# aidagroup/quad-periodic-mpc

Hardware: AMD Instinct MI355X
Metric: QP solves/sec (N=10, 13-state, 12-force) at batch=65536; 1/2/4/8 GPU (higher is better)
Workload: dtype f32

## Files before the change

### quad-periodic-mpc_amd/csrc/cmpc_class1.hip

```cpp
#include <stdlib.h>

#include "cmpc_common.h"

#ifndef CMPC_W1_WAVES_60
#define CMPC_W1_WAVES_60 4
#endif
#ifndef CMPC_W1_WAVES_PER_EU
#define CMPC_W1_WAVES_PER_EU 4
#endif
#ifndef CMPC_C1_RL
#define CMPC_C1_RL 0
#endif
#ifndef CMPC_TRIP_PRIO_AT
#define CMPC_TRIP_PRIO_AT 0
#endif
#ifndef CMPC_C1_TRIP_PRIO
#define CMPC_C1_TRIP_PRIO 2
#endif
#ifndef C1_PIPE_GRP
#define C1_PIPE_GRP 4
#endif
#ifndef CMPC_C1_CHOL2
#define CMPC_C1_CHOL2 1
#endif
// ... 51 lines not shown
template <int NV>
struct C1Geo {
  static constexpr int NG = NV / 4;
  static constexpr int PSZ = 4 * NG * NV - 8 * NG * (NG - 1);
  __host__ __device__ static constexpr int prow(int r) {
    return 4 * (r >> 2) * NV - 8 * (r >> 2) * ((r >> 2) - 1) + (r & 3) * (NV - 4 * (r >> 2));
  }
  __host__ __device__ static constexpr int prow0(int r) { return prow(r) - (r & ~3); }
  __host__ __device__ static constexpr int tri(int r) { return r * NV - ((r * (r + 1)) >> 1); }
  static_assert(NV * NV - ((NV * (NV + 1)) >> 1) <= 4 * NG * NV - 8 * NG * (NG - 1), "exchange fits P");
};
__device__ __forceinline__ int rcol(int j) { return (j * (j + 1)) >> 1; }
constexpr int rinv_cols(int words) {
  int q = 0;
  while ((q + 1) * (q + 2) <= words) q++;
  return q;
}

constexpr int OFF_E = 0;
constexpr int OFF_ZE = OFF_E + 16 * MAXN;
constexpr int OFF_REC = OFF_ZE + 16 * MAXN;

constexpr int C1_MAXFS = 24;

template <int NV>
struct SharedC1 {
  static_assert(NV % 4 == 0 && NV <= NL, "row width");
  static_assert(NV * (NV + 1) / 2 <= C1Geo<NV>::PSZ, "R must fit in P");
  static_assert(OFF_REC + CMPC_REC_WORDS(MAXN) <= C1Geo<NV>::PSZ, "prep scratch must fit in P");
  static_assert(3 * C1_MAXFS >= NV, "stance list");
  static_assert(NV * (NV + 1) / 2 <= C1Geo<NV>::PSZ - NL, "vbuf in P's tail");
  __device__ __forceinline__ float* vbuf() { return &P[C1Geo<NV>::PSZ - NL]; }
  static constexpr int QI = rinv_cols(C1Geo<NV>::PSZ - NL);
  static constexpr int RB = C1Geo<NV>::PSZ - NL - QI * (QI + 1) / 2;
  static_assert(QI * (QI + 1) / 2 <= RB, "R and R^-1 side by side");
  float P[C1Geo<NV>::PSZ];
  union {
    float BdtT[12][16];
    float ibuf[NL];
    struct {
      float bufA[NL], bufB[NL];
      float cs[2 * NL];
    } gi;
  } u;
  float sub[C1_MAXFS];
  int sfs[C1_MAXFS];
  int blkbase[MAXN + 2];
  unsigned char varblk[NL], varcol[NL];
  unsigned char cmask[NL];
};

__device__ __forceinline__ void lsync() {
  __builtin_amdgcn_wave_barrier();
  asm volatile("" ::: "memory");
}

__device__ __forceinline__ float fdiv(float a, float b) { return a * fast_rcp(b); }

template <int M>
__device__ __forceinline__ void pin(float (&x)[M]) {
#pragma unroll
  for (int c = 0; c < M; c++) asm volatile("" : "+v"(x[c]));
}

template <int LO, int HI, int MA>
__device__ __forceinline__ float pick_col(const float (&x)[MA], int q) {
  static_assert(0 <= LO && LO < HI && HI <= MA, "column range");
  if constexpr (HI - LO == 1) {
    float r = x[LO];
    asm volatile("" : "+v"(r));
    return r;
  } else {
    constexpr int MID = (LO + HI) / 2;
    if (q < MID) return pick_col<LO, MID>(x, q);
    return pick_col<MID, HI>(x, q);
  }
}

#ifndef CMPC_FENCE_COLS
#define CMPC_FENCE_COLS 16
#endif
#define CMPC_SWEEP_FENCE(c)                                                                  \
  do {                                                                                       \
    if (((c) & (CMPC_FENCE_COLS - 1)) == CMPC_FENCE_COLS - 4) __builtin_amdgcn_sched_barrier(0); \
  } while (0)

template <int NV>
__device__ __forceinline__ void solve_c1(const float* __restrict__ rec, const KParams& P,
                                         SharedC1<NV>& sh, float* __restrict__ fout,
                                         uint8_t* __restrict__ st_out, int32_t* __restrict__ it_out,
                                         int* __restrict__ ovf_list, int* __restrict__ ovf_count,
                                         int inst) {
  using G = C1Geo<NV>;
  const int v = threadIdx.x;
  const int N = P.N;
#ifdef CMPC_PHASE_PROF
  unsigned long long ph[16] = {0, 0, 0, 0, 0, 0, 0, 0, 0, 0, 0, 0, 0, 0, 0, 0};
  unsigned long long t_sub = 0;
  unsigned long long t_last = clock64();
#endif
  {
    const float4* src = reinterpret_cast<const float4*>(rec);
    float4* dst = reinterpret_cast<float4*>(&sh.P[OFF_REC]);
    for (int t = v; t < (P.rec_words >> 2); t += 64) dst[t] = src[t];
  }
  lsync();
  const float* srec = &sh.P[OFF_REC];
  const unsigned char* gait = reinterpret_cast<const unsigned char*>(srec + CMPC_REC_HDR + 12 * N);
  int nfs = 0;
  unsigned long long msk0 = 0ull, msk1 = 0ull;
  for (int c0 = 0; c0 < 4 * N; c0 += 64) {
    const int t = c0 + v;
    float ub = 0.f;
    bool f = false;
    if (t < 4 * N) {
      ub = (float)gait[t] * P.f_max;
      f = !(ub < 0.01f && ub > -0.01f);
    }
    const unsigned long long m = __ballot(f);
    if (c0 == 0) msk0 = m; else msk1 = m;
    const int pre = __popcll(m & ((1ull << v) - 1ull));
    if (f && nfs + pre < C1_MAXFS) {
      sh.sfs[nfs + pre] = t;
      sh.sub[nfs + pre] = ub;
    }
    nfs += __popcll(m);
  }
  const int n = 3 * nfs;
  if (n > NV) {
    if (v == 0 && ovf_list) ovf_list[atomicAdd(ovf_count, 1)] = inst;
    return;
  }
  lsync();
  {
    int kb = 0, kc = 0;
    if (v < n) {
      const int fs = sh.sfs[v / 3];
      kb = fs >> 2;
      kc = 3 * (fs & 3) + v % 3;
    }
    sh.varblk[v] = (unsigned char)kb;
    sh.varcol[v] = (unsigned char)kc;
    if (v <= N) {
      const int b0 = 4 * v, b1 = 4 * v - 64;
      const unsigned long long lo = (b0 >= 64) ? msk0 : (msk0 & ((1ull << b0) - 1ull));
      const unsigned long long hi = (b1 <= 0) ? 0ull : (msk1 & ((1ull << b1) - 1ull));
      sh.blkbase[v] = 3 * (__popcll(lo) + __popcll(hi));
    }
    for (int t = v; t < nfs; t += 64) sh.cmask[t] = 0;
  }
  Model md;
  make_model(srec, P.dt, md);
  make_bdt<64>(srec, md, v, sh.u.BdtT);
  lsync();
  if (v < N) {
    float e[13];
    state_error(srec, md, v, srec + CMPC_REC_HDR + 12 * v, e);
#pragma unroll
    for (int j = 0; j < 13; j++) sh.P[OFF_E + 16 * v + j] = e[j];
  }
  lsync();
  float wts[13];
#pragma unroll
  for (int j = 0; j < 12; j++) wts[j] = P.wts[j];
  wts[12] = 0.f;
  {
    float ze[13];
#pragma unroll
    for (int j = 0; j < 13; j++) ze[j] = 0.f;
    for (int i = N - 1; i >= 0; i--) {
      float e[13];
#pragma unroll
      for (int j = 0; j < 13; j++) e[j] = sh.P[OFF_E + 16 * i + j];
      recur(md, wts, e, ze);
      float mine = 0.f;
#pragma unroll
      for (int j = 0; j < 13; j++) mine = (v == j) ? ze[j] : mine;
      if (v < 13) sh.P[OFF_ZE + 16 * i + v] = mine;
    }
  }
  lsync();
  C1_MARK(0);

  const bool real = v < n;
  float gv;
  {
    const int kv = real ? sh.varblk[v] : 0;
    const int cv = real ? sh.varcol[v] : 0;
    float b[13], u1[13], u2[13];
#pragma unroll
    for (int j = 0; j < 13; j++) b[j] = real ? sh.u.BdtT[cv][j] : 0.f;
    n1_mul(md, b, u1);
    n1_mul(md, u1, u2);
    {
      float zk[13];
#pragma unroll
      for (int j = 0; j < 13; j++) zk[j] = sh.P[OFF_ZE + 16 * kv + j];
      gv = real ? 2.f * dot13(b, zk) : 0.f;
    }
    lsync();
    const int myrow = G::tri(v);
    float z[13];
#pragma unroll
    for (int j = 0; j < 13; j++) z[j] = 0.f;
    for (int i = N - 1; i >= 0; i--) {
      const bool act = real && (i >= kv);
      const float k = (float)(i - kv);
      const float k2 = 0.5f * k * (k - 1.f);
      float gk[13];
#pragma unroll
      for (int j = 0; j < 13; j++) gk[j] = act ? fmaf(k2, u2[j], fmaf(k, u1[j], b[j])) : 0.f;
      recur(md, wts, gk, z);
      asm volatile("" ::: "memory");
      const int wb = __builtin_amdgcn_readfirstlane(sh.blkbase[i]);
      step_columns(sh.u.BdtT, step_mask(msk0, msk1, i), wb, z, [&](int w, float val) {
        if (w == v) val += P.alpha2;
        if (act && w >= v) sh.P[myrow + w] = val;
      });
    }
  }
  lsync();
  C1_MARK(1);

  float slot[NV + 1];
  {
    const int vv = (v < NV) ? v : 0;
    const int myrow = G::tri(vv);
    static_for<0, NV>([&](auto C) {
      constexpr int c = decltype(C)::value;
      const int addr = (c >= vv) ? myrow + c : G::tri(c) + vv;
      const float x = sh.P[addr];
      slot[c] = (real && c < n) ? x : ((c == v) ? 1.f : 0.f);
      if ((c & 7) == 7) __builtin_amdgcn_sched_barrier(0);
    });
    slot[NV] = gv;
  }
  lsync();

  int status = CMPC_OK;
  float my_inv = 1.f;
#if CMPC_C1_CHOL2
  float i0n = 1.f, betan = 0.f, i1n = 1.f, g0n = 0.f, g1n = 0.f;
  auto look = [&](auto JJ) {
    constexpr int j = decltype(JJ)::value, j1 = j + 1;
    constexpr int cj = j & ~3, cj1 = j1 & ~3;
    if constexpr (j1 < NV) {
    float d0 = rl(slot[j], j);
    const float h10 = rl(slot[j], j1);
    if (!(d0 > 0.f)) { status = CMPC_NOT_PD; d0 = 1e-30f; }
    i0n = __builtin_amdgcn_rsqf(d0);
    betan = h10 * (i0n * i0n);
    float d1 = fmaf(-h10, betan, rl(slot[j1], j1));
    if (!(d1 > 0.f)) { status = CMPC_NOT_PD; d1 = 1e-30f; }
    i1n = __builtin_amdgcn_rsqf(d1);
    g0n = rl(slot[NV], j);
    g1n = fmaf(-betan, g0n, rl(slot[NV], j1));
    const float s1 = fmaf(-slot[j], betan, slot[j1]);
#if CMPC_C1_FUSEDJ
    g0n = -g0n * i0n;
    g1n = -g1n * i1n;
    if (v >= cj && v < NV) sh.P[G::prow(j) + v - cj] = (v >= j) ? -slot[j] * i0n : 0.f;
    if (v >= cj1 && v < NV) sh.P[G::prow(j1) + v - cj1] = (v >= j1) ? -s1 * i1n : 0.f;
#else
    if (v >= cj && v < NV) sh.P[G::prow(j) + v - cj] = (v >= j) ? slot[j] : 0.f;
    if (v >= cj1 && v < NV) sh.P[G::prow(j1) + v - cj1] = (v >= j1) ? s1 : 0.f;
#endif
    lsync();
    }
  };
  if (n > 0) look(std::integral_constant<int, 0>{});
  float jc2 = 0.f, jc3 = 0.f;
  (void)jc2; (void)jc3;
  float xunc = 0.f;
  (void)xunc;
  static_for<0, NV / 2>([&](auto KB) {
    constexpr int k = 2 * decltype(KB)::value;
    constexpr int k1 = k + 1, k2 = k + 2;
    constexpr int c0 = k & ~3, c1 = k1 & ~3, c2 = k2 & ~3;
    constexpr int rk = G::prow(k), rk1 = G::prow(k1);
    if (k < n) {
      const float i0 = i0n, beta = betan, i1 = i1n, g0 = g0n, g1 = g1n;
#if CMPC_C1_FUSEDJ
      if (v == k) my_inv = i0;
      if (v == k1) my_inv = i1;
      const float s0 = slot[k];
      const float s1 = fmaf(-s0, beta, slot[k1]);
      const float a0 = (v > k) ? s0 * i0 : 0.f;
      const float a1 = (v > k1) ? s1 * i1 : 0.f;
#else
      if (v == k) { my_inv = i0; sh.u.ibuf[k] = i0; }
      if (v == k1) { my_inv = i1; sh.u.ibuf[k1] = i1; }
      const float s0 = slot[k];
      const float s1 = fmaf(-s0, beta, slot[k1]);
      const float a0 = (v > k) ? -s0 * (i0 * i0) : 0.f;
      const float a1 = (v > k1) ? -s1 * (i1 * i1) : 0.f;
#endif
      slot[NV] = fmaf(a1, g1, fmaf(a0, g0, slot[NV]));
      static_for<c2 / 4, NV / 4>([&](auto JC) {
        constexpr int c = 4 * decltype(JC)::value;
        const float4 r0 = *reinterpret_cast<const float4*>(&sh.P[rk + c - c0]);
        const float4 r1 = *reinterpret_cast<const float4*>(&sh.P[rk1 + c - c1]);
        axpy4(a0, r0, slot[c + 0], slot[c + 1], slot[c + 2], slot[c + 3]);
        axpy4(a1, r1, slot[c + 0], slot[c + 1], slot[c + 2], slot[c + 3]);
        if constexpr (k2 < NV && c == c2) {
          if (k2 < n) look(std::integral_constant<int, k2>{});
        }
        CMPC_SWEEP_FENCE(c);
      });
#if CMPC_C1_FUSEDJ == 2
      if constexpr ((k & 3) == 0) {
        f2v t0 = {(v == k) ? 1.f : 0.f, 0.f}, t1 = {(v == k1) ? 1.f : 0.f, 0.f};
        f2v t2 = {(v == k + 2) ? 1.f : 0.f, 0.f}, t3 = {(v == k + 3) ? 1.f : 0.f, 0.f};
#if CMPC_C1_JPIPE
        piped_sweep<0, k, 1>(
            [&](auto C) {
              constexpr int q = decltype(C)::value;
              return F4x4{*reinterpret_cast<const float4*>(&sh.P[G::prow(q) + k - q]),
                          *reinterpret_cast<const float4*>(&sh.P[G::prow(q + 1) + k - q]),
                          *reinterpret_cast<const float4*>(&sh.P[G::prow(q + 2) + k - q]),
                          *reinterpret_cast<const float4*>(&sh.P[G::prow(q + 3) + k - q])};
            },
            [&](auto C, F4x4 l) {
              constexpr int q = decltype(C)::value;
              const float4 la = l.a, lb = l.b, lc = l.c, ld = l.d;
#else
        static_for<0, k / 4>([&](auto QC) {
          constexpr int q = 4 * decltype(QC)::value;
          const float4 la = *reinterpret_cast<const float4*>(&sh.P[G::prow(q) + k - q]);
          const float4 lb = *reinterpret_cast<const float4*>(&sh.P[G::prow(q + 1) + k - q]);
          const float4 lc = *reinterpret_cast<const float4*>(&sh.P[G::prow(q + 2) + k - q]);
          const float4 ld = *reinterpret_cast<const float4*>(&sh.P[G::prow(q + 3) + k - q]);
#endif
          t0.x = fmaf(slot[q], la.x, t0.x); t1.x = fmaf(slot[q], la.y, t1.x);
          t2.x = fmaf(slot[q], la.z, t2.x); t3.x = fmaf(slot[q], la.w, t3.x);
          t0.y = fmaf(slot[q + 1], lb.x, t0.y); t1.y = fmaf(slot[q + 1], lb.y, t1.y);
          t2.y = fmaf(slot[q + 1], lb.z, t2.y); t3.y = fmaf(slot[q + 1], lb.w, t3.y);
          t0.x = fmaf(slot[q + 2], lc.x, t0.x); t1.x = fmaf(slot[q + 2], lc.y, t1.x);
          t2.x = fmaf(slot[q + 2], lc.z, t2.x); t3.x = fmaf(slot[q + 2], lc.w, t3.x);
          t0.y = fmaf(slot[q + 3], ld.x, t0.y); t1.y = fmaf(slot[q + 3], ld.y, t1.y);
          t2.y = fmaf(slot[q + 3], ld.z, t2.y); t3.y = fmaf(slot[q + 3], ld.w, t3.y);
#if CMPC_C1_JPIPE
            });
#else
          __builtin_amdgcn_sched_barrier(0);
        });
#endif
        const float hk = sh.P[G::prow(k) + k1 - (k & ~3)];
        const float xk = (t0.x + t0.y) * i0;
        slot[k] = xk;
        slot[k1] = fmaf(xk, hk, t1.x + t1.y) * i1;
#if CMPC_C1_XUNC
        xunc = fmaf(slot[k1], g1, fmaf(xk, g0, xunc));
#endif
        jc2 = t2.x + t2.y;
        jc3 = t3.x + t3.y;
        asm volatile("" : "+v"(jc2), "+v"(jc3));
      } else {
        constexpr int km = k - 2;
        const float2 l0 = *reinterpret_cast<const float2*>(&sh.P[G::prow(km) + k - (km & ~3)]);
        const float2 l1 = *reinterpret_cast<const float2*>(&sh.P[G::prow(km + 1) + k - (km & ~3)]);
        const float hk = sh.P[G::prow(k) + k1 - (k & ~3)];
        const float e0 = fmaf(slot[km + 1], l1.x, fmaf(slot[km], l0.x, jc2));
        const float e1 = fmaf(slot[km + 1], l1.y, fmaf(slot[km], l0.y, jc3));
        const float xk = e0 * i0;
        slot[k] = xk;
        slot[k1] = fmaf(xk, hk, e1) * i1;
#if CMPC_C1_XUNC
        xunc = fmaf(slot[k1], g1, fmaf(xk, g0, xunc));
// ... 485 lines not shown
```

### quad-periodic-mpc_amd/csrc/cmpc_common.h

```cpp
#pragma once
#include <hip/hip_runtime.h>
#include <stdint.h>

#include <type_traits>

#include "cmpc_kernels.h"

namespace cmpc {
namespace {

constexpr int MAXN = CMPC_MAX_HORIZON;
constexpr float kBigF = 3.0e38f;

__device__ __forceinline__ float rl(float x, int lane) {
  return __int_as_float(__builtin_amdgcn_readlane(__float_as_int(x), lane));
}
__device__ __forceinline__ int rli(int x, int lane) { return __builtin_amdgcn_readlane(x, lane); }

constexpr int kDppQuadSwap1 = 0xB1;
constexpr int kDppQuadSwap2 = 0x4E;
constexpr int kDppRowShl = 0x100;
constexpr int kDppRowShr = 0x110;
constexpr int kDppWaveShl1 = 0x130;
constexpr int kDppWaveShr1 = 0x138;
// ... 60 lines not shown
__device__ __forceinline__ float lane_next(float old, float v) { return dppf<kDppWaveShl1>(old, v); }
__device__ __forceinline__ int lane_next_i(int old, int v) { return dppi<kDppWaveShl1>(old, v); }

__device__ __forceinline__ int tid_opq() {
  int x = threadIdx.x;
  asm volatile("" : "+v"(x));
  return x;
}

#ifndef CMPC_LANE_ASM
#define CMPC_LANE_ASM 1
#endif
__device__ __forceinline__ int lane_opq() {
#if CMPC_LANE_ASM
  int x;
  asm volatile("v_mbcnt_lo_u32_b32 %0, -1, 0\n\tv_mbcnt_hi_u32_b32 %0, -1, %0" : "=v"(x));
#else
  int x = (int)__builtin_amdgcn_mbcnt_hi(~0u, __builtin_amdgcn_mbcnt_lo(~0u, 0u));
  asm volatile("" : "+v"(x));
#endif
  return x;
}

template <int I, int E, class F>
__device__ __forceinline__ void static_for(F&& f) {
  if constexpr (I < E) {
    f(std::integral_constant<int, I>{});
    static_for<I + 1, E>(f);
  }
}
template <int C0, int CE, int GRP, class Ld, class F>
__device__ __forceinline__ void piped_sweep(Ld&& ld, F&& f) {
  constexpr int NCH = (CE > C0) ? (CE - C0) / 4 : 0;
  if constexpr (NCH > 0) {
    using T = decltype(ld(std::integral_constant<int, C0>{}));
    constexpr int NG = (NCH + GRP - 1) / GRP;
    T cur[GRP], nxt[GRP];
    static_for<0, GRP>([&](auto I) {
      constexpr int ch = decltype(I)::value;
      if constexpr (ch < NCH) cur[ch] = ld(std::integral_constant<int, C0 + 4 * ch>{});
    });
    static_for<0, NG>([&](auto GI) {
      constexpr int g = decltype(GI)::value;
      static_for<0, GRP>([&](auto I) {
        constexpr int ch = (g + 1) * GRP + decltype(I)::value;
        if constexpr (ch < NCH) nxt[decltype(I)::value] = ld(std::integral_constant<int, C0 + 4 * ch>{});
      });
      __builtin_amdgcn_sched_barrier(0);
      static_for<0, GRP>([&](auto I) {
        constexpr int ch = g * GRP + decltype(I)::value;
        if constexpr (ch < NCH) f(std::integral_constant<int, C0 + 4 * ch>{}, cur[decltype(I)::value]);
      });
      __builtin_amdgcn_sched_barrier(0);
      static_for<0, GRP>([&](auto I) { cur[decltype(I)::value] = nxt[decltype(I)::value]; });
    });
  }
}
struct F4x2 {
  float4 a, b;
};
struct F4x4 {
  float4 a, b, c, d;
};

__device__ __forceinline__ float vopq(float x) {
  asm volatile("" : "+v"(x));
  return x;
}
__device__ __forceinline__ float sopq(float x) {
  asm volatile("" : "+s"(x));
  return x;
}
__device__ __forceinline__ float rfl(float x) {
  return __int_as_float(__builtin_amdgcn_readfirstlane(__float_as_int(x)));
}
__device__ __forceinline__ int opaque(int x) {
  x = __builtin_amdgcn_readfirstlane(x);
  asm volatile("" : "+s"(x));
  return x;
}
__device__ __forceinline__ float fast_rcp(float x) { return __builtin_amdgcn_rcpf(x); }

typedef float f2v __attribute__((ext_vector_type(2)));
__device__ __forceinline__ void axpy4(float a, float4 r, float& x0, float& x1, float& x2, float& x3) {
  x0 = fmaf(a, r.x, x0);
  x1 = fmaf(a, r.y, x1);
  x2 = fmaf(a, r.z, x2);
  x3 = fmaf(a, r.w, x3);
}
__device__ __forceinline__ void dot4(f2v& acc, float x0, float x1, float x2, float x3, float4 r) {
  acc.x = fmaf(x0, r.x, acc.x);
  acc.x = fmaf(x1, r.y, acc.x);
  acc.x = fmaf(x2, r.z, acc.x);
  acc.x = fmaf(x3, r.w, acc.x);
}
__device__ __forceinline__ void dot4x2(f2v& acc, float x0, float x1, float x2, float x3, float4 r) {
  acc.x = fmaf(x0, r.x, acc.x);
  acc.y = fmaf(x1, r.y, acc.y);
  acc.x = fmaf(x2, r.z, acc.x);
  acc.y = fmaf(x3, r.w, acc.y);
}

__device__ __forceinline__ void wsync() {
  __builtin_amdgcn_fence(__ATOMIC_RELEASE, "workgroup");
  __builtin_amdgcn_wave_barrier();
  __builtin_amdgcn_fence(__ATOMIC_ACQUIRE, "workgroup");
}

struct Model {
  float R[9];
  float n1r[9];
  float dt, dth, xdrag;
};

__device__ __forceinline__ void n1_mul(const Model& m, const float* x, float* y) {
#pragma unroll
  for (int i = 0; i < 3; i++) y[i] = m.n1r[i * 3 + 0] * x[6] + m.n1r[i * 3 + 1] * x[7] + m.n1r[i * 3 + 2] * x[8];
  y[3] = m.dt * x[9];
  y[4] = m.dt * x[10];
  y[5] = m.dt * x[11] + (m.dth * m.xdrag) * x[9] + m.dth * x[12];
#pragma unroll
  for (int i = 6; i < 11; i++) y[i] = 0.f;
  y[11] = (m.dt * m.xdrag) * x[9] + m.dt * x[12];
  y[12] = 0.f;
}

__device__ __forceinline__ void recur(const Model& m, const float* wts, const float* e, float* z) {
  float t[13];
#pragma unroll
  for (int j = 0; j < 13; j++) t[j] = z[j];
  const float c6 = m.n1r[0] * t[0] + m.n1r[3] * t[1] + m.n1r[6] * t[2];
  const float c7 = m.n1r[1] * t[0] + m.n1r[4] * t[1] + m.n1r[7] * t[2];
  const float c8 = m.n1r[2] * t[0] + m.n1r[5] * t[1] + m.n1r[8] * t[2];
  const float c9 = m.dt * t[3] + (m.dt * m.xdrag) * t[11] + (m.dth * m.xdrag) * t[5];
  const float c10 = m.dt * t[4];
  const float c11 = m.dt * t[5];
  const float c12 = m.dt * t[11] + m.dth * t[5];
#pragma unroll
  for (int j = 0; j < 13; j++) z[j] = wts[j] * e[j] + t[j];
  z[6] += c6; z[7] += c7; z[8] += c8; z[9] += c9; z[10] += c10; z[11] += c11; z[12] += c12;
}

__device__ __forceinline__ float dot13(const float* a, const float* b) {
  float s = 0.f;
#pragma unroll
  for (int j = 0; j < 13; j++) s = fmaf(a[j], b[j], s);
  return s;
}

__device__ __forceinline__ unsigned step_mask(unsigned long long m0, unsigned long long m1, int i) {
  return (unsigned)(((i < 16) ? (m0 >> (4 * i)) : (m1 >> (4 * i - 64))) & 15ull);
}

template <class St>
__device__ __forceinline__ void step_columns(const float (*BdtT)[16], unsigned mi, int wb,
                                             const float* z, St&& st) {
  int w = wb;
  static_for<0, 4>([&](auto F) {
    constexpr int f = decltype(F)::value;
    if (mi & (1u << f)) {
      static_for<0, 3>([&](auto A) {
        constexpr int c = 3 * f + decltype(A)::value;
        float bw[16];
#pragma unroll
        for (int q = 0; q < 4; q++) {
          const float4 b4 = *reinterpret_cast<const float4*>(&BdtT[c][4 * q]);
          bw[4 * q] = b4.x; bw[4 * q + 1] = b4.y; bw[4 * q + 2] = b4.z; bw[4 * q + 3] = b4.w;
        }
        st(w, 2.f * dot13(bw, z));
        w++;
      });
    }
  });
}

__device__ __forceinline__ void make_model(const float* __restrict__ rec, float dt, Model& md) {
  const float qw = rec[CMPC_REC_Q + 0], qx = rec[CMPC_REC_Q + 1], qy = rec[CMPC_REC_Q + 2],
              qz = rec[CMPC_REC_Q + 3];
  const float tx = 2.f * qx, ty = 2.f * qy, tz = 2.f * qz;
  const float twx = tx * qw, twy = ty * qw, twz = tz * qw;
  const float txx = tx * qx, txy = ty * qx, txz = tz * qx;
  const float tyy = ty * qy, tyz = tz * qy, tzz = tz * qz;
  md.R[0] = 1.f - (tyy + tzz); md.R[1] = txy - twz;         md.R[2] = txz + twy;
  md.R[3] = txy + twz;         md.R[4] = 1.f - (txx + tzz); md.R[5] = tyz - twx;
  md.R[6] = txz - twy;         md.R[7] = tyz + twx;         md.R[8] = 1.f - (txx + tyy);
  md.dt = dt;
  md.dth = dt * dt * 0.5f;
  md.xdrag = rec[CMPC_REC_XDRAG];
#pragma unroll
  for (int i = 0; i < 3; i++)
#pragma unroll
    for (int j = 0; j < 3; j++) md.n1r[i * 3 + j] = dt * md.R[j * 3 + i];
}

template <int NT>
__device__ __forceinline__ void make_bdt(const float* __restrict__ rec, const Model& md, int tid,
                                         float (*BdtT)[16]) {
  static_assert(NT >= 12, "one thread per force column");
  if (tid < 12) {
    const float Ib0 = .07f, Ib1 = 0.26f, Ib2 = 0.242f;
    float Iw[9];
#pragma unroll
    for (int i = 0; i < 3; i++)
#pragma unroll
      for (int j = 0; j < 3; j++)
        Iw[i * 3 + j] = md.R[i * 3 + 0] * Ib0 * md.R[j * 3 + 0] + md.R[i * 3 + 1] * Ib1 * md.R[j * 3 + 1] +
                        md.R[i * 3 + 2] * Ib2 * md.R[j * 3 + 2];
    const float c00 = Iw[4] * Iw[8] - Iw[5] * Iw[7];
    const float c10 = Iw[5] * Iw[6] - Iw[3] * Iw[8];
    const float c20 = Iw[3] * Iw[7] - Iw[4] * Iw[6];
    const float idet = 1.f / (Iw[0] * c00 + Iw[1] * c10 + Iw[2] * c20);
    float Ii[9];
    Ii[0] = c00 * idet; Ii[1] = (Iw[2] * Iw[7] - Iw[1] * Iw[8]) * idet; Ii[2] = (Iw[1] * Iw[5] - Iw[2] * Iw[4]) * idet;
    Ii[3] = c10 * idet; Ii[4] = (Iw[0] * Iw[8] - Iw[2] * Iw[6]) * idet; Ii[5] = (Iw[2] * Iw[3] - Iw[0] * Iw[5]) * idet;
    Ii[6] = c20 * idet; Ii[7] = (Iw[1] * Iw[6] - Iw[0] * Iw[7]) * idet; Ii[8] = (Iw[0] * Iw[4] - Iw[1] * Iw[3]) * idet;
    const float im = 1.f / 12.0f;
    const float dt = md.dt, dt2 = md.dth, dt3 = md.dt * md.dt * md.dt / 6.f;
    const int c = tid;
    const int b = c / 3, a = c - 3 * (c / 3);
    const float r0 = rec[CMPC_REC_R + 0 * 4 + b], r1 = rec[CMPC_REC_R + 1 * 4 + b],
                r2 = rec[CMPC_REC_R + 2 * 4 + b];
    const float cx0 = (a == 0) ? 0.f : (a == 1) ? -r2 : r1;
    const float cx1 = (a == 0) ? r2 : (a == 1) ? 0.f : -r0;
    const float cx2 = (a == 0) ? -r1 : (a == 1) ? r0 : 0.f;
    float T[3];
#pragma unroll
    for (int i = 0; i < 3; i++) T[i] = Ii[i * 3 + 0] * cx0 + Ii[i * 3 + 1] * cx1 + Ii[i * 3 + 2] * cx2;
    const float e0 = (a == 0) ? im : 0.f, e1 = (a == 1) ? im : 0.f, e2 = (a == 2) ? im : 0.f;
    float* col = BdtT[c];
#pragma unroll
    for (int s = 0; s < 3; s++)
      col[s] = dt2 * (md.R[0 * 3 + s] * T[0] + md.R[1 * 3 + s] * T[1] + md.R[2 * 3 + s] * T[2]);
    col[3] = dt2 * e0;
    col[4] = dt2 * e1;
    col[5] = dt2 * e2 + dt3 * md.xdrag * e0;
#pragma unroll
    for (int s = 0; s < 3; s++) col[6 + s] = dt * T[s];
    col[9] = dt * e0;
    col[10] = dt * e1;
    col[11] = dt * e2 + dt2 * md.xdrag * e0;
    col[12] = 0.f;
    col[13] = 0.f;
    col[14] = 0.f;
    col[15] = 0.f;
  }
}

template <typename RecPtr>
__device__ __forceinline__ void quat_to_rpy(RecPtr rec, float* rpy) {
  const float qw = rec[CMPC_REC_Q + 0], qx = rec[CMPC_REC_Q + 1], qy = rec[CMPC_REC_Q + 2],
              qz = rec[CMPC_REC_Q + 3];
  float as = -2.f * (qx * qz - qw * qy);
  as = fminf(as, 0.99999f);
  rpy[0] = atan2f(2.f * (qy * qz + qw * qx), qw * qw - qx * qx - qy * qy + qz * qz);
  rpy[1] = asinf(as);
  rpy[2] = atan2f(2.f * (qx * qy + qw * qz), qw * qw + qx * qx - qy * qy - qz * qz);
}

__device__ __forceinline__ void state_error(const float* __restrict__ rec, const Model& md, int i,
                                            const float* traj_i, float* e) {
  float x0[13];
  {
    quat_to_rpy(rec, x0);
#pragma unroll
    for (int k = 0; k < 3; k++) {
      x0[3 + k] = rec[CMPC_REC_P + k];
      x0[6 + k] = rec[CMPC_REC_W + k];
      x0[9 + k] = rec[CMPC_REC_V + k];
    }
    x0[12] = -9.8f;
  }
  float X1[13], X2[13], qf[13], F1[13], F2[13];
  n1_mul(md, x0, X1);
  n1_mul(md, X1, X2);
  const uint32_t flags = __float_as_uint(rec[CMPC_REC_FLAGS]);
  const float f3 = (flags & 1u) ? rec[CMPC_REC_FEST3] : 0.f;
#pragma unroll
  for (int j = 0; j < 13; j++) qf[j] = 0.f;
  qf[9] = md.dt * f3;
  qf[3] = md.dth * f3;
  qf[11] = md.dth * md.xdrag * f3;
  qf[5] = (md.dt * md.dt * md.dt / 6.f) * md.xdrag * f3;
  n1_mul(md, qf, F1);
  n1_mul(md, F1, F2);
  const float m1 = (float)(i + 1);
  const float m2 = 0.5f * m1 * (float)i;
  const float s2 = 0.5f * (float)i * (float)(i + 1);
  const float s3 = (float)(i + 1) * (float)i * (float)(i - 1) / 6.f;
#pragma unroll
  for (int j = 0; j < 13; j++) {
    float ev = x0[j] + m1 * X1[j] + m2 * X2[j] + m1 * qf[j] + s2 * F1[j] + s3 * F2[j];
    if (j < 12) ev -= traj_i[j];
    e[j] = ev;
  }
}

__device__ __forceinline__ double rl_d(double x, int lane) {
  const long long b = __double_as_longlong(x);
  const int lo = __builtin_amdgcn_readlane((int)b, lane);
  const int hi = __builtin_amdgcn_readlane((int)(b >> 32), lane);
  return __longlong_as_double(((long long)hi << 32) | (long long)(unsigned)lo);
}

struct Cons {
  int ia, iz;
  float ca, cb, bp;
};
__device__ __forceinline__ Cons decode_cons(int c, float mui, float sub_s) {
  Cons k;
  const int sft = c / 6, t = c - 6 * (c / 6);
  k.iz = 3 * sft + 2;
  if (t < 4) {
    k.ia = 3 * sft + (t >> 1);
    k.ca = (t & 1) ? -mui : mui;
    k.cb = 1.f;
    k.bp = 0.f;
  } else {
    k.ia = k.iz;
    k.ca = 0.f;
    k.cb = (t == 4) ? 1.f : -1.f;
    k.bp = (t == 4) ? 0.f : -sub_s;
  }
  return k;
}

}
}
```

### quad-periodic-mpc_amd/csrc/cmpc_condense.hip

```cpp
#include "cmpc_common.h"

namespace cmpc {
namespace {

constexpr int NTG = 256;

struct SharedC {
  float BdtT[12][16];
  float traj[12 * MAXN];
  float E[MAXN][16];
  float ZE[MAXN][16];
};

__device__ void condense_one(const float* __restrict__ rec, const KParams& P, SharedC& sh,
                             float* __restrict__ H, float* __restrict__ g) {
  const int tid = threadIdx.x;
  const int N = P.N;
  const int n = 12 * N;
  for (int t = tid; t < 12 * N; t += NTG) sh.traj[t] = rec[CMPC_REC_HDR + t];
  Model md;
  make_model(rec, P.dt, md);
  make_bdt<NTG>(rec, md, tid, sh.BdtT);
  __syncthreads();
  if (tid < N) {
    float e[13];
    state_error(rec, md, tid, &sh.traj[12 * tid], e);
#pragma unroll
    for (int j = 0; j < 13; j++) sh.E[tid][j] = e[j];
  }
  __syncthreads();
  float wts[13];
#pragma unroll
  for (int j = 0; j < 12; j++) wts[j] = P.wts[j];
  wts[12] = 0.f;
  if (tid < 64) {
    float ze[13];
#pragma unroll
    for (int j = 0; j < 13; j++) ze[j] = 0.f;
    for (int i = N - 1; i >= 0; i--) {
      float e[13];
#pragma unroll
      for (int j = 0; j < 13; j++) e[j] = sh.E[i][j];
      recur(md, wts, e, ze);
      if ((tid & 63) == 0) {
#pragma unroll
        for (int j = 0; j < 13; j++) sh.ZE[i][j] = ze[j];
      }
    }
  }
  __syncthreads();
  for (int v = tid; v < n; v += NTG) {
    const int kv = v / 12, cv = v - 12 * (v / 12);
    float b[13], u1[13], u2[13];
#pragma unroll
    for (int j = 0; j < 13; j++) b[j] = sh.BdtT[cv][j];
    n1_mul(md, b, u1);
    n1_mul(md, u1, u2);
    {
      float zk[13];
#pragma unroll
      for (int j = 0; j < 13; j++) zk[j] = sh.ZE[kv][j];
      g[v] = 2.f * dot13(b, zk);
    }
    float z[13];
#pragma unroll
    for (int j = 0; j < 13; j++) z[j] = 0.f;
    for (int i = N - 1; i >= kv; i--) {
      const float k = (float)(i - kv);
      const float k2 = 0.5f * k * (k - 1.f);
      float gk[13];
#pragma unroll
      for (int j = 0; j < 13; j++) gk[j] = fmaf(k2, u2[j], fmaf(k, u1[j], b[j]));
      recur(md, wts, gk, z);
      for (int w = max(12 * i, v); w < 12 * i + 12; w++) {
        float bw[13];
#pragma unroll
        for (int j = 0; j < 13; j++) bw[j] = sh.BdtT[w - 12 * i][j];
        float val = 2.f * dot13(bw, z);
        if (w == v) val += P.alpha2;
#ifdef CMPC_DIAG_PERTURB
        val *= 1.f + CMPC_DIAG_PERTURB;
#endif
        H[(size_t)v * n + w] = val;
        H[(size_t)w * n + v] = val;
      }
    }
  }
}

__global__ __launch_bounds__(NTG) void cmpc_condense_kernel(const float* __restrict__ recs, int batch, KParams P,
                                                            float* __restrict__ Hout, float* __restrict__ gout) {
  __shared__ SharedC sh;
  const size_t n = 12 * (size_t)P.N;
  for (int inst = blockIdx.x; inst < batch; inst += gridDim.x) {
    condense_one(recs + (size_t)inst * P.rec_words, P, sh, Hout + inst * n * n, gout + inst * n);
    __syncthreads();
  }
}

}

hipError_t launch_condense(const float* d_recs, int batch, const KParams& P, float* d_H, float* d_g,
                           hipStream_t stream) {
  if (batch <= 0) return hipSuccess;
  const int grid = batch < 2048 ? batch : 2048;
  hipLaunchKernelGGL(cmpc_condense_kernel, dim3(grid), dim3(NTG), 0, stream, d_recs, batch, P, d_H, d_g);
  return hipGetLastError();
}

}
```

### quad-periodic-mpc_amd/csrc/cmpc_tail.hip

```cpp
#include "cmpc_common.h"

#ifndef CMPC_TAIL_WAVES_PER_EU
#define CMPC_TAIL_WAVES_PER_EU 3
#endif
#ifndef CMPC_TRIP_PRIO_AT
#define CMPC_TRIP_PRIO_AT 0
#endif
#ifndef CMPC_TAIL_TRIP_PRIO
#define CMPC_TAIL_TRIP_PRIO 3
#endif
#ifndef CMPC_TAIL_DOT2
#define CMPC_TAIL_DOT2 0
#endif
#if CMPC_TAIL_DOT2
#define T_DOT dot4x2
#else
#define T_DOT dot4
#endif
#ifndef CMPC_TAIL_PRIO
#define CMPC_TAIL_PRIO 1
#endif
#ifndef TAIL_PIPE_GRP
#define TAIL_PIPE_GRP 4
#endif

#ifdef CMPC_PHASE_PROF
__device__ unsigned long long g_t_phase[16];
#define T_MARK(i)                               \
  do {                                          \
    const unsigned long long _n = clock64();    \
    ph[i] += _n - t_last;                       \
    t_last = _n;                                \
  } while (0)
#else
#define T_MARK(i) \
  do {            \
  } while (0)
#endif

namespace cmpc {
namespace {

constexpr int kTailRows = 8;

template <int T>
struct TGeo {
  static_assert(T == 8 || T == 16, "tail rows");
  static constexpr int NV = 64 + T;
  static constexpr int NG = NV / 4;
  static constexpr int PSZ = 4 * NG * NV - 8 * NG * (NG - 1);
  __host__ __device__ static constexpr int prow(int r) {
    return 4 * (r >> 2) * NV - 8 * (r >> 2) * ((r >> 2) - 1) + (r & 3) * (NV - 4 * (r >> 2));
  }
  __host__ __device__ static constexpr int tri(int r) { return r * NV - ((r * (r + 1)) >> 1); }
  static constexpr int LPR = 64 / T;
  static constexpr int TQ = T / LPR;
  static constexpr int SW = NV / LPR;
  static constexpr int MAXFS = (NV + 2) / 3;
  static_assert(NV * (NV + 1) / 2 <= PSZ, "exchange fits P");
  static_assert(64 * 65 / 2 <= PSZ - NV, "R (q <= 64) below vbuf");
};

constexpr int T_OFF_E = 0;
constexpr int T_OFF_ZE = T_OFF_E + 16 * MAXN;
constexpr int T_OFF_REC = T_OFF_ZE + 16 * MAXN;

__device__ __forceinline__ int rcol(int j) { return (j * (j + 1)) >> 1; }

constexpr int tail_rinv_cols(int words) {
  int q = 0;
  while ((q + 1) * (q + 2) <= words) q++;
  return q;
}

template <int T>
struct SharedT {
  using G = TGeo<T>;
  static_assert(T_OFF_REC + CMPC_REC_WORDS(MAXN) <= G::PSZ, "prep scratch must fit in P");
  __device__ __forceinline__ float* vbuf() { return &P[G::PSZ - G::NV]; }
  static constexpr int QI = tail_rinv_cols(G::PSZ - G::NV);
  static constexpr int RB = G::PSZ - G::NV - QI * (QI + 1) / 2;
  static_assert(QI * (QI + 1) / 2 <= RB, "R and R^-1 side by side");
  float P[G::PSZ];
  union {
    float BdtT[12][16];
    struct {
      float ibuf[G::NV];
      float bpair[G::NV / 2];
      float h22[T * T];
      float gt[T];
    } ch;
    struct {
      float bufA[G::NV], bufB[G::NV];
      float cs[2 * 64];
      float xs[G::NV];
    } gi;
  } u;
  float gtail[T];
  float sub[G::MAXFS];
  int sfs[G::MAXFS];
  int blkbase[MAXN + 2];
  unsigned char varblk[G::NV], varcol[G::NV];
  unsigned char cmask[G::MAXFS];
};

__device__ __forceinline__ void tsync() {
  __builtin_amdgcn_wave_barrier();
  asm volatile("" ::: "memory");
}

template <int M>
__device__ __forceinline__ void tpin(float (&x)[M]) {
#pragma unroll
  for (int c = 0; c < M; c++) asm volatile("" : "+v"(x[c]));
}

#define CMPC_TSWEEP_FENCE(c)                                       \
  do {                                                             \
    if (((c) & 15) == 12) __builtin_amdgcn_sched_barrier(0);       \
  } while (0)

template <int LPR>
__device__ __forceinline__ float group_sum(float v) {
  v += dppf<kDppQuadSwap1>(0.f, v);
  v += dppf<kDppQuadSwap2>(0.f, v);
  if constexpr (LPR == 8) v += dppf<kDppRowHalfMirror>(0.f, v);
  return v;
}

template <int T>
__device__ __forceinline__ void solve_t(const float* __restrict__ rec, const KParams& P,
                                        SharedT<T>& sh, float* __restrict__ fout,
                                        uint8_t* __restrict__ st_out, int32_t* __restrict__ it_out,
                                        int* __restrict__ ovf_list, int* __restrict__ ovf_count,
                                        int inst) {
  using G = TGeo<T>;
  constexpr int NV = G::NV, LPR = G::LPR, TQ = G::TQ, SW = G::SW;
  const int v = tid_opq();
  const int ti = v / LPR, ts = v % LPR;
  const int N = opaque(P.N);
#ifdef CMPC_PHASE_PROF
  unsigned long long ph[16] = {0, 0, 0, 0, 0, 0, 0, 0, 0, 0, 0, 0, 0, 0, 0, 0};
  unsigned long long t_last = clock64();
#endif
  {
    const float4* src = reinterpret_cast<const float4*>(rec);
    float4* dst = reinterpret_cast<float4*>(&sh.P[T_OFF_REC]);
    for (int t = v; t < (P.rec_words >> 2); t += 64) dst[t] = src[t];
  }
  tsync();
  const float* srec = &sh.P[T_OFF_REC];
  const unsigned char* gait = reinterpret_cast<const unsigned char*>(srec + CMPC_REC_HDR + 12 * N);
  int nfs = 0;
  unsigned long long msk0 = 0ull, msk1 = 0ull;
  for (int c0 = 0; c0 < 4 * N; c0 += 64) {
    const int t = c0 + v;
    float ub = 0.f;
    bool f = false;
    if (t < 4 * N) {
      ub = (float)gait[t] * P.f_max;
      f = !(ub < 0.01f && ub > -0.01f);
    }
    const unsigned long long m = __ballot(f);
    if (c0 == 0) msk0 = m; else msk1 = m;
    const int pre = __popcll(m & ((1ull << v) - 1ull));
    if (f && nfs + pre < G::MAXFS) {
      sh.sfs[nfs + pre] = t;
      sh.sub[nfs + pre] = ub;
    }
    nfs += __popcll(m);
  }
  const int n = 3 * nfs;
  if (n > NV || n <= 64) {
    if (v == 0) { st_out[0] = CMPC_BAD_INPUT; if (it_out) it_out[0] = 0; }
    return;
  }
  tsync();
  for (int t = v; t < NV; t += 64) {
    int kb = 0, kc = 0;
    if (t < n) {
      const int fs = sh.sfs[t / 3];
      kb = fs >> 2;
      kc = 3 * (fs & 3) + t % 3;
    }
    sh.varblk[t] = (unsigned char)kb;
    sh.varcol[t] = (unsigned char)kc;
  }
  if (v <= N) {
    const int b0 = 4 * v, b1 = 4 * v - 64;
    const unsigned long long lo = (b0 >= 64) ? msk0 : (msk0 & ((1ull << b0) - 1ull));
    const unsigned long long hi = (b1 <= 0) ? 0ull : (msk1 & ((1ull << b1) - 1ull));
    sh.blkbase[v] = 3 * (__popcll(lo) + __popcll(hi));
  }
  if (v < nfs) sh.cmask[v] = 0;
  Model md;
  make_model(srec, P.dt, md);
  make_bdt<64>(srec, md, v, sh.u.BdtT);
  tsync();
  if (v < N) {
    float e[13];
    state_error(srec, md, v, srec + CMPC_REC_HDR + 12 * v, e);
#pragma unroll
    for (int j = 0; j < 13; j++) sh.P[T_OFF_E + 16 * v + j] = e[j];
  }
  tsync();
  float wts[13];
#pragma unroll
  for (int j = 0; j < 12; j++) wts[j] = P.wts[j];
  wts[12] = 0.f;
  {
    float ze[13];
#pragma unroll
    for (int j = 0; j < 13; j++) ze[j] = 0.f;
    for (int i = N - 1; i >= 0; i--) {
      float e[13];
#pragma unroll
      for (int j = 0; j < 13; j++) e[j] = sh.P[T_OFF_E + 16 * i + j];
      recur(md, wts, e, ze);
      float mine = 0.f;
#pragma unroll
      for (int j = 0; j < 13; j++) mine = (v == j) ? ze[j] : mine;
      if (v < 13) sh.P[T_OFF_ZE + 16 * i + v] = mine;
    }
  }
  tsync();

  float gv;
  {
    const int kv = sh.varblk[v];
    const int cv = sh.varcol[v];
    float b[13], u1[13], u2[13];
#pragma unroll
    for (int j = 0; j < 13; j++) b[j] = sh.u.BdtT[cv][j];
    n1_mul(md, b, u1);
    n1_mul(md, u1, u2);
    {
      float zk[13];
#pragma unroll
      for (int j = 0; j < 13; j++) zk[j] = sh.P[T_OFF_ZE + 16 * kv + j];
      gv = 2.f * dot13(b, zk);
      const bool tr = v < T && 64 + v < n;
      const int kt = tr ? sh.varblk[64 + v] : 0, ct = tr ? sh.varcol[64 + v] : 0;
      float bt[13], zt[13];
#pragma unroll
      for (int j = 0; j < 13; j++) {
        bt[j] = sh.u.BdtT[ct][j];
        zt[j] = sh.P[T_OFF_ZE + 16 * kt + j];
      }
      const float gtl = tr ? 2.f * dot13(bt, zt) : 0.f;
      if (v < T) sh.gtail[v] = gtl;
    }
    tsync();
    const int myrow = G::tri(v);
    float z[13];
#pragma unroll
    for (int j = 0; j < 13; j++) z[j] = 0.f;
    for (int i = N - 1; i >= 0; i--) {
      const bool act = i >= kv;
      const float k = (float)(i - kv);
      const float k2 = 0.5f * k * (k - 1.f);
      float gk[13];
#pragma unroll
      for (int j = 0; j < 13; j++) gk[j] = act ? fmaf(k2, u2[j], fmaf(k, u1[j], b[j])) : 0.f;
      recur(md, wts, gk, z);
      asm volatile("" ::: "memory");
      const int wb = __builtin_amdgcn_readfirstlane(sh.blkbase[i]);
      step_columns(sh.u.BdtT, step_mask(msk0, msk1, i), wb, z, [&](int w, float val) {
        if (w == v) val += P.alpha2;
        if (act && w >= v) sh.P[myrow + w] = val;
      });
    }
  }
  {
    const int r = 64 + v;
    const bool real = v < T && r < n;
    const int kv = real ? sh.varblk[r] : 0;
    const int cv = real ? sh.varcol[r] : 0;
    const int k64 = __builtin_amdgcn_readfirstlane((int)sh.varblk[64]);
    float b[13], u1[13], u2[13];
#pragma unroll
    for (int j = 0; j < 13; j++) b[j] = sh.u.BdtT[cv][j];
    n1_mul(md, b, u1);
    n1_mul(md, u1, u2);
    const int myrow = G::tri(real ? r : 64);
    float z[13];
#pragma unroll
    for (int j = 0; j < 13; j++) z[j] = 0.f;
    for (int i = N - 1; i >= k64; i--) {
      const bool act = real && i >= kv;
      const float k = (float)(i - kv);
      const float k2 = 0.5f * k * (k - 1.f);
      float gk[13];
#pragma unroll
      for (int j = 0; j < 13; j++) gk[j] = act ? fmaf(k2, u2[j], fmaf(k, u1[j], b[j])) : 0.f;
      recur(md, wts, gk, z);
      asm volatile("" ::: "memory");
      const int wb = __builtin_amdgcn_readfirstlane(sh.blkbase[i]);
      step_columns(sh.u.BdtT, step_mask(msk0, msk1, i), wb, z, [&](int w, float val) {
        if (w == r) val += P.alpha2;
        if (act && w >= r) sh.P[myrow + w] = val;
      });
    }
  }
  tsync();

  T_MARK(0);
  float slot[NV + 1];
  {
    const int myrow = G::tri(v);
    static_for<0, NV>([&](auto C) {
      constexpr int c = decltype(C)::value;
      const int addr = (c >= v) ? myrow + c : G::tri(c) + v;
      const float x = sh.P[addr];
      if constexpr (c < 64) {
        slot[c] = x;
      } else {
        slot[c] = (c < opaque(n)) ? x : 0.f;
      }
      if ((c & 7) == 7) __builtin_amdgcn_sched_barrier(0);
    });
    slot[NV] = gv;
  }
  float tq[TQ];
  float gt;
  {
    const int r = 64 + ti;
#pragma unroll
    for (int m = 0; m < TQ; m++) {
      const int c = 64 + TQ * ts + m;
      const int addr = (c >= r) ? G::tri(r) + c : G::tri(c) + r;
      const float x = sh.P[addr];
      tq[m] = (r < n && c < n) ? x : ((r == c) ? 1.f : 0.f);
    }
    gt = (r < n) ? sh.gtail[ti] : 0.f;
  }
  tsync();

  T_MARK(1);
  int status = CMPC_OK;
  float my_inv = 1.f;
  float i0n = 1.f, betan = 0.f, i1n = 1.f, g0n = 0.f, g1n = 0.f;
  auto look = [&](auto JJ) {
    constexpr int j = decltype(JJ)::value, j1 = j + 1;
    constexpr int cj = j & ~3, cj1 = j1 & ~3;
    if constexpr (j1 < 64) {
      float d0 = rl(slot[j], j);
      const float h10 = rl(slot[j], j1);
      if (!(d0 > 0.f)) { status = CMPC_NOT_PD; d0 = 1e-30f; }
      i0n = __builtin_amdgcn_rsqf(d0);
      betan = h10 * (i0n * i0n);
      float d1 = fmaf(-h10, betan, rl(slot[j1], j1));
      if (!(d1 > 0.f)) { status = CMPC_NOT_PD; d1 = 1e-30f; }
      i1n = __builtin_amdgcn_rsqf(d1);
      g0n = rl(slot[NV], j);
      g1n = fmaf(-betan, g0n, rl(slot[NV], j1));
      const float s1 = fmaf(-slot[j], betan, slot[j1]);
      if (v >= cj) sh.P[G::prow(j) + v - cj] = (v >= j) ? slot[j] : 0.f;
      if (v >= cj1) sh.P[G::prow(j1) + v - cj1] = (v >= j1) ? s1 : 0.f;
      tsync();
    }
  };
  auto pub_tail = [&](auto JJ) {
    constexpr int j = decltype(JJ)::value, j1 = j + 1;
    constexpr int bj = G::prow(j) + 64 - (j & ~3), bj1 = G::prow(j1) + 64 - (j1 & ~3);
    {
      float x = 0.f;
      static_for<0, T>([&](auto M) {
        constexpr int m = decltype(M)::value;
        const float a = rl(slot[64 + m], j), b = rl(slot[64 + m], j1);
        x = (v == m) ? a : x;
        x = (v == T + m) ? b : x;
      });
      if (v < 2 * T) sh.P[(v < T) ? bj + v : bj1 + v - T] = x;
    }
  };
  look(std::integral_constant<int, 0>{});
  pub_tail(std::integral_constant<int, 0>{});
  tsync();
  static_for<0, 32>([&](auto KB) {
    constexpr int k = 2 * decltype(KB)::value;
    constexpr int k1 = k + 1, k2 = k + 2;
    constexpr int c0 = k & ~3, c1 = k1 & ~3, c2 = k2 & ~3;
    constexpr int rk = G::prow(k), rk1 = G::prow(k1);
    const float i0 = i0n, beta = betan, i1 = i1n, g0 = g0n, g1 = g1n;
    if (v == k) { my_inv = i0; sh.u.ch.ibuf[k] = i0; }
    if (v == k1) { my_inv = i1; sh.u.ch.ibuf[k1] = i1; }
    if (v == 0) sh.u.ch.bpair[k / 2] = beta;
    const float s0 = slot[k];
    const float s1 = fmaf(-s0, beta, slot[k1]);
    const float a0 = (v > k) ? -s0 * (i0 * i0) : 0.f;
    const float a1 = (v > k1) ? -s1 * (i1 * i1) : 0.f;
    slot[NV] = fmaf(a1, g1, fmaf(a0, g0, slot[NV]));
    static_for<c2 / 4, 16>([&](auto JC) {
      constexpr int c = 4 * decltype(JC)::value;
      const float4 r0 = *reinterpret_cast<const float4*>(&sh.P[rk + c - c0]);
      const float4 r1 = *reinterpret_cast<const float4*>(&sh.P[rk1 + c - c1]);
      axpy4(a0, r0, slot[c + 0], slot[c + 1], slot[c + 2], slot[c + 3]);
      axpy4(a1, r1, slot[c + 0], slot[c + 1], slot[c + 2], slot[c + 3]);
      if constexpr (k2 < 64 && c == c2) look(std::integral_constant<int, k2>{});
      CMPC_TSWEEP_FENCE(c);
    });
    tpin(slot);
    {
      const float a0t = fmaf(-beta, a1, a0);
      static_for<16, NV / 4>([&](auto JC) {
        constexpr int c = 4 * decltype(JC)::value;
        const float4 r0 = *reinterpret_cast<const float4*>(&sh.P[rk + c - c0]);
        const float4 r1 = *reinterpret_cast<const float4*>(&sh.P[rk1 + c - c1]);
        axpy4(a0t, r0, slot[c + 0], slot[c + 1], slot[c + 2], slot[c + 3]);
        axpy4(a1, r1, slot[c + 0], slot[c + 1], slot[c + 2], slot[c + 3]);
      });
      tpin(slot);
      const float h0 = sh.P[rk + 64 + ti - c0], h1 = sh.P[rk1 + 64 + ti - c1];
      const float s1t = fmaf(-h0, beta, h1);
      const float a1r = -s1t * (i1 * i1);
      const float a0c = -h0 * (i0 * i0);
      const float a0r = fmaf(-beta, a1r, a0c);
#pragma unroll
      for (int m = 0; m < TQ; m++) {
        const float p0 = sh.P[rk + 64 + TQ * ts + m - c0], p1 = sh.P[rk1 + 64 + TQ * ts + m - c1];
        tq[m] = fmaf(a1r, p1, fmaf(a0r, p0, tq[m]));
      }
      gt = fmaf(a1r, g1, fmaf(a0c, g0, gt));
    }
    if constexpr (k2 < 64) pub_tail(std::integral_constant<int, k2>{});
    tsync();
    tpin(slot);
    tpin(tq);
    asm volatile("" : "+v"(gt));
  });

  T_MARK(2);
  float yt = 0.f;
  {
#pragma unroll
    for (int m = 0; m < TQ; m++) sh.u.ch.h22[ti * T + TQ * ts + m] = tq[m];
    if (ts == 0) sh.u.ch.gt[ti] = gt;
    tsync();
    float trow[T];
    const int li = (v < T) ? v : 0;
    static_for<0, T>([&](auto C) {
      constexpr int c = decltype(C)::value;
      trow[c] = (v < T) ? sh.u.ch.h22[li * T + c] : 0.f;
    });
    float gti = (v < T) ? sh.u.ch.gt[li] : 0.f;
    float tinv = 1.f;
    tsync();
    static_for<0, T>([&](auto TT) {
      constexpr int t = decltype(TT)::value;
      constexpr int k = 64 + t, ck = k & ~3, rk = G::prow(k);
      if (v < T && v >= ck - 64) sh.P[rk + 64 + v - ck] = (v >= t) ? trow[t] : 0.f;
// ... 555 lines not shown
```

Measured before the change: 48.17 million.

## Compute Hessian step entries via structured B projection instead of dense dot13

Replaces the per-column 13-element dot products against the shared-memory B matrix with a factored form. It projects z once per step through the rotation, inverse inertia and mass terms, then forms each force column's three entries with a cross product against foot positions. It also exploits sparsity in the column-power expansion (col_power) so that only the nonzero terms of u1/u2 are used. Shared-memory loads and FMAs per Hessian entry drop, at the cost of extra per-thread registers for CondGeo and possible float rounding differences. The tail kernel keeps the old dot13 path by default.

```diff
diff --git a/quad-periodic-mpc_amd/csrc/cmpc_class1.hip b/quad-periodic-mpc_amd/csrc/cmpc_class1.hip
--- a/quad-periodic-mpc_amd/csrc/cmpc_class1.hip
+++ b/quad-periodic-mpc_amd/csrc/cmpc_class1.hip
@@ -227,6 +227,8 @@
   Model md;
   make_model(srec, P.dt, md);
   make_bdt<64>(srec, md, v, sh.u.BdtT);
+  CondGeo cg;
+  make_cond_geo<true>(srec, md, cg);
   lsync();
   if (v < N) {
     float e[13];
@@ -283,12 +285,13 @@
       const float k = (float)(i - kv);
       const float k2 = 0.5f * k * (k - 1.f);
       float gk[13];
-#pragma unroll
-      for (int j = 0; j < 13; j++) gk[j] = act ? fmaf(k2, u2[j], fmaf(k, u1[j], b[j])) : 0.f;
+      col_power(b, u1, u2, k, k2, gk);
+#pragma unroll
+      for (int j = 0; j < 13; j++) gk[j] = act ? gk[j] : 0.f;
       recur(md, wts, gk, z);
       asm volatile("" ::: "memory");
       const int wb = __builtin_amdgcn_readfirstlane(sh.blkbase[i]);
-      step_columns(sh.u.BdtT, step_mask(msk0, msk1, i), wb, z, [&](int w, float val) {
+      step_entries(md, cg, sh.u.BdtT, step_mask(msk0, msk1, i), wb, z, [&](int w, float val) {
         if (w == v) val += P.alpha2;
         if (act && w >= v) sh.P[myrow + w] = val;
       });
diff --git a/quad-periodic-mpc_amd/csrc/cmpc_common.h b/quad-periodic-mpc_amd/csrc/cmpc_common.h
--- a/quad-periodic-mpc_amd/csrc/cmpc_common.h
+++ b/quad-periodic-mpc_amd/csrc/cmpc_common.h
@@ -236,9 +236,100 @@
   return (unsigned)(((i < 16) ? (m0 >> (4 * i)) : (m1 >> (4 * i - 64))) & 15ull);
 }
 
+#ifndef CMPC_COND_DOT13
+#define CMPC_COND_DOT13 0
+#endif
+
+struct CondGeo {
+  float Ii[9];
+  float r[12];
+};
+struct StepProj {
+  float w[3], p[3];
+};
+
+__device__ __forceinline__ void make_iinv(const Model& md, float* Ii) {
+  const float Ib0 = .07f, Ib1 = 0.26f, Ib2 = 0.242f;
+  float Iw[9];
+#pragma unroll
+  for (int i = 0; i < 3; i++)
+#pragma unroll
+    for (int j = 0; j < 3; j++)
+      Iw[i * 3 + j] = md.R[i * 3 + 0] * Ib0 * md.R[j * 3 + 0] + md.R[i * 3 + 1] * Ib1 * md.R[j * 3 + 1] +
+                      md.R[i * 3 + 2] * Ib2 * md.R[j * 3 + 2];
+  const float c00 = Iw[4] * Iw[8] - Iw[5] * Iw[7];
+  const float c10 = Iw[5] * Iw[6] - Iw[3] * Iw[8];
+  const float c20 = Iw[3] * Iw[7] - Iw[4] * Iw[6];
+  const float idet = 1.f / (Iw[0] * c00 + Iw[1] * c10 + Iw[2] * c20);
+  Ii[0] = c00 * idet; Ii[1] = (Iw[2] * Iw[7] - Iw[1] * Iw[8]) * idet; Ii[2] = (Iw[1] * Iw[5] - Iw[2] * Iw[4]) * idet;
+  Ii[3] = c10 * idet; Ii[4] = (Iw[0] * Iw[8] - Iw[2] * Iw[6]) * idet; Ii[5] = (Iw[2] * Iw[3] - Iw[0] * Iw[5]) * idet;
+  Ii[6] = c20 * idet; Ii[7] = (Iw[1] * Iw[6] - Iw[0] * Iw[7]) * idet; Ii[8] = (Iw[0] * Iw[4] - Iw[1] * Iw[3]) * idet;
+}
+
+template <bool UNIFORM, typename RecPtr>
+__device__ __forceinline__ void make_cond_geo(RecPtr rec, const Model& md, CondGeo& cg) {
+  make_iinv(md, cg.Ii);
+#pragma unroll
+  for (int j = 0; j < 12; j++) cg.r[j] = rec[CMPC_REC_R + j];
+  if constexpr (UNIFORM) {
+#pragma unroll
+    for (int j = 0; j < 9; j++) cg.Ii[j] = rfl(cg.Ii[j]);
+#pragma unroll
+    for (int j = 0; j < 12; j++) cg.r[j] = rfl(cg.r[j]);
+  }
+}
+
+__device__ __forceinline__ void step_proj(const Model& md, const CondGeo& cg, const float* z, StepProj& pj) {
+  const float dt2 = 2.f * md.dt, dtq = 2.f * md.dth, dtc = md.dt * md.dt * md.dt / 3.f;
+  const float im = 1.f / 12.0f;
+  float q[3];
+#pragma unroll
+  for (int i = 0; i < 3; i++)
+    q[i] = fmaf(dt2, z[6 + i], dtq * fmaf(md.R[i * 3 + 2], z[2], fmaf(md.R[i * 3 + 1], z[1], md.R[i * 3] * z[0])));
+#pragma unroll
+  for (int j = 0; j < 3; j++)
+    pj.w[j] = fmaf(cg.Ii[6 + j], q[2], fmaf(cg.Ii[3 + j], q[1], cg.Ii[j] * q[0]));
+#pragma unroll
+  for (int a = 0; a < 3; a++) pj.p[a] = im * fmaf(dt2, z[9 + a], dtq * z[3 + a]);
+  pj.p[0] = fmaf(im * md.xdrag, fmaf(dtq, z[11], dtc * z[5]), pj.p[0]);
+}
+
+__device__ __forceinline__ void foot_entries(const StepProj& pj, float r0, float r1, float r2, float* out) {
+  out[0] = fmaf(pj.w[1], r2, fmaf(-pj.w[2], r1, pj.p[0]));
+  out[1] = fmaf(pj.w[2], r0, fmaf(-pj.w[0], r2, pj.p[1]));
+  out[2] = fmaf(pj.w[0], r1, fmaf(-pj.w[1], r0, pj.p[2]));
+}
+
+__device__ __forceinline__ void col_power(const float* b, const float* u1, const float* u2, float k, float k2,
+                                          float* e) {
+#pragma unroll
+  for (int j = 0; j < 5; j++) e[j] = fmaf(k, u1[j], b[j]);
+  e[5] = fmaf(k2, u2[5], fmaf(k, u1[5], b[5]));
+#pragma unroll
+  for (int j = 6; j < 11; j++) e[j] = b[j];
+  e[11] = fmaf(k, u1[11], b[11]);
+  e[12] = b[12];
+}
+
 template <class St>
-__device__ __forceinline__ void step_columns(const float (*BdtT)[16], unsigned mi, int wb,
-                                             const float* z, St&& st) {
+__device__ __forceinline__ void step_columns(const CondGeo& cg, unsigned mi, int wb, const StepProj& pj,
+                                             St&& st) {
+  int w = wb;
+  static_for<0, 4>([&](auto F) {
+    constexpr int f = decltype(F)::value;
+    if (mi & (1u << f)) {
+      float val[3];
+      foot_entries(pj, cg.r[f], cg.r[4 + f], cg.r[8 + f], val);
+      st(w, val[0]);
+      st(w + 1, val[1]);
+      st(w + 2, val[2]);
+      w += 3;
+    }
+  });
+}
+template <class St>
+__device__ __forceinline__ void step_columns_dot13(const float (*BdtT)[16], unsigned mi, int wb,
+                                                   const float* z, St&& st) {
   int w = wb;
   static_for<0, 4>([&](auto F) {
     constexpr int f = decltype(F)::value;
@@ -256,6 +347,17 @@
       });
     }
   });
+}
+template <class St>
+__device__ __forceinline__ void step_entries(const Model& md, const CondGeo& cg, const float (*BdtT)[16],
+                                             unsigned mi, int wb, const float* z, St&& st) {
+#if CMPC_COND_DOT13
+  step_columns_dot13(BdtT, mi, wb, z, st);
+#else
+  StepProj pj;
+  step_proj(md, cg, z, pj);
+  step_columns(cg, mi, wb, pj, st);
+#endif
 }
 
 __device__ __forceinline__ void make_model(const float* __restrict__ rec, float dt, Model& md) {
@@ -282,22 +384,8 @@
                                          float (*BdtT)[16]) {
   static_assert(NT >= 12, "one thread per force column");
   if (tid < 12) {
-    const float Ib0 = .07f, Ib1 = 0.26f, Ib2 = 0.242f;
-    float Iw[9];
-#pragma unroll
-    for (int i = 0; i < 3; i++)
-#pragma unroll
-      for (int j = 0; j < 3; j++)
-        Iw[i * 3 + j] = md.R[i * 3 + 0] * Ib0 * md.R[j * 3 + 0] + md.R[i * 3 + 1] * Ib1 * md.R[j * 3 + 1] +
-                        md.R[i * 3 + 2] * Ib2 * md.R[j * 3 + 2];
-    const float c00 = Iw[4] * Iw[8] - Iw[5] * Iw[7];
-    const float c10 = Iw[5] * Iw[6] - Iw[3] * Iw[8];
-    const float c20 = Iw[3] * Iw[7] - Iw[4] * Iw[6];
-    const float idet = 1.f / (Iw[0] * c00 + Iw[1] * c10 + Iw[2] * c20);
     float Ii[9];
-    Ii[0] = c00 * idet; Ii[1] = (Iw[2] * Iw[7] - Iw[1] * Iw[8]) * idet; Ii[2] = (Iw[1] * Iw[5] - Iw[2] * Iw[4]) * idet;
-    Ii[3] = c10 * idet; Ii[4] = (Iw[0] * Iw[8] - Iw[2] * Iw[6]) * idet; Ii[5] = (Iw[2] * Iw[3] - Iw[0] * Iw[5]) * idet;
-    Ii[6] = c20 * idet; Ii[7] = (Iw[1] * Iw[6] - Iw[0] * Iw[7]) * idet; Ii[8] = (Iw[0] * Iw[4] - Iw[1] * Iw[3]) * idet;
+    make_iinv(md, Ii);
     const float im = 1.f / 12.0f;
     const float dt = md.dt, dt2 = md.dth, dt3 = md.dt * md.dt * md.dt / 6.f;
     const int c = tid;
diff --git a/quad-periodic-mpc_amd/csrc/cmpc_condense.hip b/quad-periodic-mpc_amd/csrc/cmpc_condense.hip
--- a/quad-periodic-mpc_amd/csrc/cmpc_condense.hip
+++ b/quad-periodic-mpc_amd/csrc/cmpc_condense.hip
@@ -21,6 +21,8 @@
   Model md;
   make_model(rec, P.dt, md);
   make_bdt<NTG>(rec, md, tid, sh.BdtT);
+  CondGeo cg;
+  make_cond_geo<true>(rec, md, cg);
   __syncthreads();
   if (tid < N) {
     float e[13];
@@ -69,21 +71,18 @@
       const float k = (float)(i - kv);
       const float k2 = 0.5f * k * (k - 1.f);
       float gk[13];
-#pragma unroll
-      for (int j = 0; j < 13; j++) gk[j] = fmaf(k2, u2[j], fmaf(k, u1[j], b[j]));
+      col_power(b, u1, u2, k, k2, gk);
       recur(md, wts, gk, z);
-      for (int w = max(12 * i, v); w < 12 * i + 12; w++) {
-        float bw[13];
-#pragma unroll
-        for (int j = 0; j < 13; j++) bw[j] = sh.BdtT[w - 12 * i][j];
-        float val = 2.f * dot13(bw, z);
+      step_entries(md, cg, sh.BdtT, 15u, 12 * i, z, [&](int w, float val) {
         if (w == v) val += P.alpha2;
 #ifdef CMPC_DIAG_PERTURB
         val *= 1.f + CMPC_DIAG_PERTURB;
 #endif
-        H[(size_t)v * n + w] = val;
-        H[(size_t)w * n + v] = val;
-      }
+        if (w >= v) {
+          H[(size_t)v * n + w] = val;
+          H[(size_t)w * n + v] = val;
+        }
+      });
     }
   }
 }
diff --git a/quad-periodic-mpc_amd/csrc/cmpc_tail.hip b/quad-periodic-mpc_amd/csrc/cmpc_tail.hip
--- a/quad-periodic-mpc_amd/csrc/cmpc_tail.hip
+++ b/quad-periodic-mpc_amd/csrc/cmpc_tail.hip
@@ -1,3 +1,7 @@
+
+#ifndef CMPC_COND_DOT13
+#define CMPC_COND_DOT13 1
+#endif
 #include "cmpc_common.h"
 
 #ifndef CMPC_TAIL_WAVES_PER_EU
@@ -225,6 +229,8 @@
   }
   tsync();
 
+  CondGeo cg;
+  make_cond_geo<true>(srec, md, cg);
   float gv;
   {
     const int kv = sh.varblk[v];
@@ -260,12 +266,13 @@
       const float k = (float)(i - kv);
       const float k2 = 0.5f * k * (k - 1.f);
       float gk[13];
-#pragma unroll
-      for (int j = 0; j < 13; j++) gk[j] = act ? fmaf(k2, u2[j], fmaf(k, u1[j], b[j])) : 0.f;
+      col_power(b, u1, u2, k, k2, gk);
+#pragma unroll
+      for (int j = 0; j < 13; j++) gk[j] = act ? gk[j] : 0.f;
       recur(md, wts, gk, z);
       asm volatile("" ::: "memory");
       const int wb = __builtin_amdgcn_readfirstlane(sh.blkbase[i]);
-      step_columns(sh.u.BdtT, step_mask(msk0, msk1, i), wb, z, [&](int w, float val) {
+      step_entries(md, cg, sh.u.BdtT, step_mask(msk0, msk1, i), wb, z, [&](int w, float val) {
         if (w == v) val += P.alpha2;
         if (act && w >= v) sh.P[myrow + w] = val;
       });
@@ -291,12 +298,13 @@
       const float k = (float)(i - kv);
       const float k2 = 0.5f * k * (k - 1.f);
       float gk[13];
-#pragma unroll
-      for (int j = 0; j < 13; j++) gk[j] = act ? fmaf(k2, u2[j], fmaf(k, u1[j], b[j])) : 0.f;
+      col_power(b, u1, u2, k, k2, gk);
+#pragma unroll
+      for (int j = 0; j < 13; j++) gk[j] = act ? gk[j] : 0.f;
       recur(md, wts, gk, z);
       asm volatile("" ::: "memory");
       const int wb = __builtin_amdgcn_readfirstlane(sh.blkbase[i]);
-      step_columns(sh.u.BdtT, step_mask(msk0, msk1, i), wb, z, [&](int w, float val) {
+      step_entries(md, cg, sh.u.BdtT, step_mask(msk0, msk1, i), wb, z, [&](int w, float val) {
         if (w == r) val += P.alpha2;
         if (act && w >= r) sh.P[myrow + w] = val;
       });
```

Result: faster. 50.14 million, median of 6 (+4.1%).
